# SRainGit/CAE-LO

Measured on AMD Instinct MI355X. Metric: KITTI frames/sec end-to-end (keypts+desc+match+RANSAC), higher is better.
Workload: dtype f32

## Files before the change

### cae-lo_amd/csrc/caelo_internal.h

```cpp
#pragma once
#include <hip/hip_runtime.h>
#include <stdint.h>
#include <stdio.h>
#include <string.h>

#include "../../include/caelo.h"

#define CAELO_API extern "C" __attribute__((visibility("default")))

void caelo_set_error(const char *fmt, ...);

#define CAELO_HIP(expr)                                                                     \
    do {                                                                                    \
        hipError_t _e = (expr);                                                             \
        if (_e != hipSuccess) {                                                             \
            caelo_set_error("%s:%d: %s failed: %s", __FILE__, __LINE__, #expr, hipGetErrorString(_e)); \
            return CAELO_ERR_HIP;                                                           \
        }                                                                                   \
    } while (0)

#define CAELO_LAUNCH_CHECK()                                                                \
    do {                                                                                    \
        hipError_t _e = hipGetLastError();                                                  \
        if (_e != hipSuccess) {                                                             \
            caelo_set_error("%s:%d: kernel launch failed: %s", __FILE__, __LINE__, hipGetErrorString(_e)); \
            return CAELO_ERR_HIP;                                                           \
        }                                                                                   \
    } while (0)

#define CAELO_REQUIRE(cond, msg)                         \
    do {                                                 \
        if (!(cond)) {                                   \
            caelo_set_error("%s: %s", __func__, msg);    \
            return CAELO_ERR_ARG;                        \
        }                                                \
    } while (0)

struct caelo_ctx {
    int device;
    float *resp_w;
    bool has_resp;
    float *enc_w1;
    float *enc_b1;
    float *enc_w2;
    float *enc_b2;
    float *enc_c0;
    float *enc_w3;
    float *enc_b3;
    void *enc_w1f;
    void *enc_w2x;
    void *enc_w3x;
    void *enc_wd1x;
    float *enc_bd1;
    float *enc_wd2;
    void *enc_wd2q;
    float *enc_bd2;
    void *enc32_wd1x;
    float *enc32_bd1;
    bool has_enc;
    int enc_hidden, enc_code;
    bool enc_reference;
    int32_t *faults;
    double *proj_edge;
    float *dec_w;
    bool has_dec;
    int dec_hidden, dec_out;
    double calib_angle;
};

#define CAELO_EMPTY_KEY 0xFFFFFFFFFFFFFFFFull

struct caelo_brick_table {
    unsigned long long *keys;
    unsigned long long *bits;
    uint32_t mask;
};

struct caelo_kd;
struct caelo_voxmap {
    int64_t max_points;
    caelo_kd *kd;
    bool order_tracked;
    bool kd_lists;
    caelo_brick_table brick[3];
    unsigned long long *vkeys[3];
    uint32_t *vfirst[3];
    uint32_t vmask[3];
    int32_t *counts;
    uint32_t *list0, *list1;
    unsigned long long *sp_keys, *sb_keys;
    uint32_t *sp_first, *sb_cnt;
    uint4 *sp_list;
    uint32_t sp_mask;
    size_t sp_off, sp_bytes;
    char *base;
    size_t ff_bytes_keys, ff_bytes_min, ff_bytes_all, zero_off, zero_bytes, total_bytes;
    bool lists_valid;
    void *scratch;
    int64_t scratch_bytes;
    char *xo_base;
    size_t xo_bytes;
    int xo_frames;
    float *corr;
};

void kd_destroy(caelo_voxmap *m);
void seqloader_rings(const caelo_seqloader *L, int *ring_batches, int *keep_batches);
int kd_store_lists(caelo_voxmap *m, const int16_t *const lists[3], const int64_t ns[3], hipStream_t s);
int kd_begin_device_lists(caelo_voxmap *m, int16_t *vox_out[3], int32_t **n_out, hipStream_t s);
int kd_resolve(const caelo_voxmap *m, const float *pts, int pts_ld, int64_t k_max, const int32_t *n_key, uint64_t *bits, uint8_t *flags,
               hipStream_t s);
int kd_resolve_many(int n, const caelo_voxmap *const *maps, const float *const *pts, int pts_ld, int64_t k_max, const int32_t *const *n_key,
                    uint64_t *const *bits, uint8_t *const *flags, hipStream_t s, bool queues_clear = false);
#define KD_ST_CENSUS 20
int kd_fused_storage(caelo_voxmap *m, int16_t *vox_out[3], int32_t **state_out);
int kd_report_left(int n, const caelo_voxmap *const *maps, int32_t *const *status, hipStream_t s);

struct SuspectTables {
    unsigned long long *sp_keys, *sb_keys;
    uint32_t *sp_first, *sb_cnt;
    uint4 *list;
    uint32_t mask;
};
inline SuspectTables suspect_tables(const caelo_voxmap *m) {
    return SuspectTables{m->sp_keys, m->sb_keys, m->sp_first, m->sb_cnt, m->sp_list, m->sp_mask};
}

#ifndef CAELO_FB_MAX
#define CAELO_FB_MAX 8
#endif
struct DedupScratch;
struct caelo_frame_dev {
    const float *pc;
    int64_t n;
    int32_t pc_stride, dist_c;
    float *ring;
    int32_t *counter, *winner;
    float *resp;
    unsigned long long *cand;
    int32_t *cand_count;
    unsigned long long *kp_elig;
    int64_t *key_pixels;
    float *key_pts, *valid;
    int32_t *n_key;
    uint8_t *flags;
    int32_t *status;
    int32_t kp_ld, valid_ld;
    caelo_brick_table brick[3];
    int32_t *counts;
    uint32_t *list0, *list1;
    SuspectTables sp;
    unsigned long long *vkeys[3];
    uint32_t *vfirst[3];
    uint32_t vmask0, vmask12;
    unsigned long long *bits;
    DedupScratch *dd;
};
struct caelo_frame_set {
    caelo_frame_dev f[CAELO_FB_MAX];
    int32_t n;
};
static_assert(sizeof(caelo_frame_set) <= 3800, "caelo_frame_set must fit the kernel argument segment");
void frame_dev_set_map(caelo_frame_dev &d, const caelo_voxmap *m);

struct caelo_pair_dev {
    const float *f0, *f1;
    const int32_t *n0, *n1;
    const float *pc0, *pc1;
    int64_t *pair_idx;
    void *ws_match, *ws_ransac;
    const double *rand;
    caelo_pose_result *result;
    uint8_t *mask;
    caelo_ransac_cert *cert;
    int32_t cert_only;
};
struct caelo_pair_set {
    caelo_pair_dev p[CAELO_FB_MAX];
    int32_t n;
    int32_t *faults;
};
int match_set(const caelo_pair_set &ps, int ld0, int64_t k0_max, int ld1, int64_t k1_max, int dim, hipStream_t s);
int ransac_set(const caelo_pair_set &ps, int pld0, int pld1, int64_t k1_max, hipStream_t s);
struct caelo_adaptive_table {
    const float *rows;
    const int32_t *n_key, *pairs;
    const int64_t *pair_idx;
    const double *draws;
    double threshold;
    caelo_adaptive_result *result;
    uint8_t *mask;
    int64_t n_pairs;
};
int adaptive_table(const caelo_adaptive_table &at, hipStream_t s);
int certify_record(const caelo_ransac_cert &c, const double *rnd, caelo_pose_result *res, uint8_t *mask, int64_t mask_len, int32_t *evals);

struct caelo_clear_item {
    void *ptr;
    size_t bytes;
    uint32_t pattern;
};
#define CAELO_CLEAR_MAX 12
struct caelo_clear_list {
    caelo_clear_item item[CAELO_CLEAR_MAX];
    int n;
};
int caelo_clear_many(const caelo_clear_list &list, hipStream_t s);
int caelo_clear_many_set(const caelo_clear_list *lists, int n_frames, hipStream_t s);

int ring_project_launch(caelo_ctx *c, const float *pc, int64_t n, float *ring, int32_t *counter, int32_t *winner, int32_t *status,
                        hipStream_t s);
int ring_respond_launch(caelo_ctx *c, const float *in, int in_w, int in_c, float *resp, hipStream_t s);
int ring_keypoints_launch(const float *ring, int ring_w, int ring_c, int dist_c, const int32_t *counter, int cnt_w,
                          const float *resp, unsigned long long *cand, int32_t *cand_count,
                          int64_t *key_pixels, float *key_pts, int kp_ld, float *valid, int valid_ld, int32_t *n_key,
                          int32_t *status, hipStream_t s);
int ring_project_set(caelo_ctx *c, const caelo_frame_set &fs, hipStream_t s);
int ring_respond_set(caelo_ctx *c, const caelo_frame_set &fs, int in_w, int in_c, hipStream_t s, int row0, int rows);
int ring_keypoints_set(const caelo_frame_set &fs, int ring_w, int ring_c, int cnt_w, hipStream_t s);
int ring_keypoints_select_set(const caelo_frame_set &fs, int ring_w, int ring_c, hipStream_t s);
int front_fused_set(caelo_ctx *c, caelo_voxmap *const *maps, const caelo_frame_set &fs, hipStream_t s);
void vox_clear_items(caelo_voxmap *m, int level, caelo_clear_list &list);
int vox_clear_for_fast_build(caelo_voxmap *m, caelo_clear_list &list, hipStream_t s);
int vox_clear_for_fast_build_set(caelo_voxmap *const *maps, int n, caelo_clear_list *lists, hipStream_t s);
int vox_build_fast_set(caelo_voxmap *const *maps, const caelo_frame_set &fs, hipStream_t s);
int vox_build_set(caelo_voxmap *const *maps, const caelo_frame_set &fs, bool track_order, hipStream_t s);
int vox_patches_set(const caelo_frame_set &fs, int64_t k_max, bool check_counts, hipStream_t s);
int dedup_set(const caelo_frame_set &fs, bool enabled, hipStream_t s);
int vox_build_launch(caelo_voxmap *m, const float *pc, int64_t n, int stride, bool track_order, int32_t *status,
                     hipStream_t s);
int vox_build_fast_launch(caelo_voxmap *m, const float *pc, int64_t n, int stride, int32_t *status, hipStream_t s);
int vox_patches_launch(const caelo_voxmap *m, const float *pts, int pts_ld, int64_t k_max, const int32_t *n_key,
                       uint64_t *bits, uint8_t *flags, int32_t *status, bool check_counts, hipStream_t s,
                       void *dedup_scratch = nullptr);
#define CAELO_FRAME_PATCHES (CAELO_MAX_KEYPTS * 3)
struct caelo_dedup_tables {
    int32_t count;
    int32_t pad[63];
    int32_t list[CAELO_FRAME_PATCHES];
    int32_t slot_of[CAELO_FRAME_PATCHES];
};
#define CAELO_FRAME_BITS_BYTES ((size_t)CAELO_FRAME_PATCHES * 64 * 8)
#define CAELO_FRAME_BUF_BYTES (CAELO_FRAME_BITS_BYTES + sizeof(caelo_dedup_tables))
__host__ __device__ inline caelo_dedup_tables *caelo_frame_tables(const uint64_t *frame_bits) {
    return (caelo_dedup_tables *)((char *)frame_bits + CAELO_FRAME_BITS_BYTES);
}
#define DD_SLOTS_FRAME 8192
#define DD_SLOTS_SET 65536
#define DD_EMPTY 0xFFFFFFFFFFFFFFFFull
struct DedupScratch {
    unsigned long long table[DD_SLOTS_SET];
    int32_t pslot[CAELO_FRAME_PATCHES];
    int32_t rep[CAELO_FRAME_PATCHES];
};
__host__ __device__ inline uint32_t dedup_slot_mask(int n_frames) { return (n_frames > 1 ? DD_SLOTS_SET : DD_SLOTS_FRAME) - 1; }
int64_t dedup_scratch_bytes();
void dedup_clear_item(void *scratch, int n_frames, caelo_clear_list &list);
unsigned long long dedup_hash_mask();
bool dedup_enabled(int mode);
int dedup_launch(uint64_t *frame_bits, void *scratch, bool enabled, hipStream_t s);

#define CAELO_ENC_MAX_FRAMES CAELO_FB_MAX
struct caelo_enc_out {
    float *base[CAELO_ENC_MAX_FRAMES];
    int64_t per_frame;
};
#define CAELO_ENC_WS_HEADER 4096
#define CAELO_ENC_WS_MFMA 3072
struct caelo_enc_in {
    const unsigned long long *bits;
    int64_t frame_stride;
    int32_t per_frame, n_frames, dedup;
    int32_t yield;
};
__device__ inline const caelo_dedup_tables *enc_tables(const caelo_enc_in &in, int f) {
    return (const caelo_dedup_tables *)(in.bits + (size_t)f * in.frame_stride + (size_t)in.per_frame * 64);
}
int encode_batch_impl(caelo_ctx *c, const uint64_t *bits, int64_t n_patches, int group, const caelo_enc_out &outs,
                      int out_stride, void *ws, hipStream_t s, hipEvent_t *ev, const caelo_enc_in *in = nullptr);
int64_t enc_dense_pad(int64_t n);
int enc_upload_dense1(const float *wd1, const float *bd1, int K, void **wx_dev, float **bd_dev);
int64_t enc_dense32_part_bytes(int64_t np);
void enc_dense32_slices(int64_t *used, int64_t *sized);
int enc_dense32_head_launch(caelo_ctx *c, const float *f3, int64_t n_patches, int64_t np, float *part, int group, float *out,
                            int out_stride, hipStream_t s);
int encode_impl(caelo_ctx *c, const uint64_t *bits, int64_t n_patches, int group, float *out, int out_stride, void *ws,
                hipStream_t s, hipEvent_t *ev);

struct caelo_extract_args {
    caelo_ctx *ctx;
    caelo_voxmap *map;
    const float *pc;
    int64_t n;
    int dist_channels, mode;
    float *key_pts;
    int kp_ld;
    float *features;
    int feat_ld;
    float *valid;
    int valid_ld;
    int64_t *key_pixels;
    int32_t *n_key;
    uint8_t *flags;
    int32_t *status;
    void *ws;
    uint64_t *bits;
};
int extract_check(const caelo_extract_args &a);
int extract_front_launch(const caelo_extract_args &a, hipStream_t s);
int extract_front_set(const caelo_extract_args *args, int n, hipStream_t s, hipStream_t s_vox = nullptr, hipEvent_t ev_fork = nullptr,
                      hipEvent_t ev_join = nullptr);
int extract_encode_launch(const caelo_extract_args &a, hipStream_t s);
int exact_patches_prepare(caelo_voxmap *const *maps, int n_frames);
void exact_patches_clear_item(caelo_voxmap *m, caelo_clear_list &list);
int exact_patches_redo(caelo_voxmap *const *maps, const caelo_frame_set &fs, const caelo_extract_args *args, int n, hipStream_t s);

int correct_prepare(caelo_voxmap *const *maps, int n);
int correct_set(const caelo_extract_args *args, int n, hipStream_t s);

#define CAELO_KP_HIST_BINS 2048

typedef float f32x4 __attribute__((ext_vector_type(4)));
#define MFMA16(a, b, c) __builtin_amdgcn_mfma_f32_16x16x4f32((a), (b), (c), 0, 0, 0)

__device__ inline void caelo_frame_block(int n_frames, unsigned &frame, unsigned &block, unsigned &per_frame) {
    per_frame = gridDim.x / (unsigned)n_frames;
    if ((n_frames & (n_frames - 1)) == 0) {
        frame = blockIdx.x & (unsigned)(n_frames - 1);
        block = blockIdx.x / (unsigned)n_frames;
    } else {
        frame = blockIdx.x / per_frame;
        block = blockIdx.x - frame * per_frame;
    }
}

__device__ inline void caelo_lds_barrier() { __asm__ volatile("s_waitcnt lgkmcnt(0)\n\ts_barrier" ::: "memory"); }

__host__ __device__ inline unsigned long long caelo_pack3(int x, int y, int z) {
    return ((unsigned long long)(unsigned)(x & 0xFFFFF) << 40) | ((unsigned long long)(unsigned)(y & 0xFFFFF) << 20) |
           (unsigned long long)(unsigned)(z & 0xFFFFF);
}

__device__ inline uint32_t caelo_hash64(unsigned long long k) {
    k ^= k >> 33;
    k *= 0xff51afd7ed558ccdULL;
    k ^= k >> 33;
    k *= 0xc4ceb9fe1a85ec53ULL;
    k ^= k >> 33;
    return (uint32_t)k;
}

__device__ inline unsigned long long caelo_dd_mix(unsigned long long k) {
    k ^= k >> 33;
    k *= 0xff51afd7ed558ccdULL;
    k ^= k >> 33;
    k *= 0xc4ceb9fe1a85ec53ULL;
    k ^= k >> 33;
    return k;
}
__device__ inline void caelo_dedup_insert(unsigned long long word, int lane, int p, int gp, DedupScratch *S, DedupScratch *T, uint32_t slot_mask,
                                          unsigned long long hash_mask) {
    unsigned long long h = caelo_dd_mix(word + 0x9E3779B97F4A7C15ull * (unsigned)(lane + 1));
#pragma unroll
    for (int o = 32; o > 0; o >>= 1) h += __shfl_xor(h, o);
    if (lane != 0) return;
    h = caelo_dd_mix(h) & hash_mask & 0xFFFFFFFFFEull;
    const unsigned long long mine = (h << 24) | (unsigned)gp;
    uint32_t slot = (uint32_t)caelo_dd_mix(h) & slot_mask;
    for (;;) {
        const unsigned long long cur = atomicCAS(&T->table[slot], DD_EMPTY, mine);
        if (cur == DD_EMPTY) break;
        if ((cur >> 24) == h) {
            if (mine < cur) atomicMin(&T->table[slot], mine);
            break;
        }
        slot = (slot + 1) & slot_mask;
    }
    S->pslot[p] = (int32_t)slot;
}

__device__ inline int caelo_brick_find(const caelo_brick_table &t, unsigned long long key) {
    uint32_t h = caelo_hash64(key) & t.mask;
    for (uint32_t probe = 0; probe <= t.mask; ++probe) {
        const unsigned long long k = t.keys[h];
        if (k == key) return (int)h;
        if (k == CAELO_EMPTY_KEY) return -1;
        h = (h + 1) & t.mask;
    }
    return -1;
}

static inline hipStream_t caelo_stream(void *s) { return (hipStream_t)s; }

#include <mutex>
#define CAELO_MAX_DEVICES 64
template <typename T, typename F>
static T per_device_once(int device, T (&slot)[CAELO_MAX_DEVICES], bool (&have)[CAELO_MAX_DEVICES], std::mutex &mu, F make) {
    const int d = device >= 0 && device < CAELO_MAX_DEVICES ? device : 0;
    std::lock_guard<std::mutex> lock(mu);
    if (!have[d]) { slot[d] = make(); have[d] = true; }
    return slot[d];
}

#ifdef __HIPCC__
__device__ inline int caelo_block_reserve(int32_t *gcounter, bool pred, int *s_tmp) {
    const int lane = threadIdx.x & 63;
    if (threadIdx.x == 0) s_tmp[0] = 0;
    __syncthreads();
    const unsigned long long m = __ballot(pred);
    int wbase = 0;
    if (m && lane == __ffsll((long long)m) - 1) wbase = atomicAdd(&s_tmp[0], __popcll(m));
    if (m) wbase = __shfl(wbase, __ffsll((long long)m) - 1);
    __syncthreads();
    if (threadIdx.x == 0) s_tmp[1] = s_tmp[0] ? atomicAdd(gcounter, s_tmp[0]) : 0;
    __syncthreads();
    return s_tmp[1] + wbase + __popcll(m & ((1ull << lane) - 1ull));
}
__device__ inline int caelo_block_reserve_async(int32_t *gcounter, bool pred, int *s_tmp) {
    const int lane = threadIdx.x & 63;
    if (threadIdx.x == 0) s_tmp[0] = 0;
    caelo_lds_barrier();
    const unsigned long long m = __ballot(pred);
    int wbase = 0;
    if (m && lane == __ffsll((long long)m) - 1) wbase = atomicAdd(&s_tmp[0], __popcll(m));
    if (m) wbase = __shfl(wbase, __ffsll((long long)m) - 1);
    caelo_lds_barrier();
    if (threadIdx.x == 0) s_tmp[1] = s_tmp[0] ? atomicAdd(gcounter, s_tmp[0]) : 0;
    caelo_lds_barrier();
    return s_tmp[1] + wbase + __popcll(m & ((1ull << lane) - 1ull));
}
__device__ inline void caelo_block_add(int32_t *gcounter, int value, int *s_tmp) {
    if (threadIdx.x == 0) s_tmp[0] = 0;
    __syncthreads();
#pragma unroll
    for (int o = 32; o > 0; o >>= 1) value += __shfl_xor(value, o);
    if ((threadIdx.x & 63) == 0 && value) atomicAdd(&s_tmp[0], value);
    __syncthreads();
    if (threadIdx.x == 0 && s_tmp[0]) atomicAdd(gcounter, s_tmp[0]);
}
#endif
```

### cae-lo_amd/csrc/voxel_front.inc

```
#pragma once

#define VOX_SIZE 0.02
#define BLOCK_REAL 1.28
#define VIS_L 99.84
#define VIS_W 99.84
#define VIS_H 14.72

__device__ inline int table_insert(unsigned long long *keys, uint32_t mask, unsigned long long key) {
    uint32_t h = caelo_hash64(key) & mask;
    for (uint32_t probe = 0; probe <= mask; ++probe) {
        unsigned long long k = keys[h];
        if (k == key) return (int)h;
        if (k == CAELO_EMPTY_KEY) {
            k = atomicCAS(&keys[h], CAELO_EMPTY_KEY, key);
            if (k == CAELO_EMPTY_KEY || k == key) return (int)h;
        }
        h = (h + 1) & mask;
    }
    return -1;
}

__device__ inline int table_find(const unsigned long long *keys, uint32_t mask, unsigned long long key) {
    uint32_t h = caelo_hash64(key) & mask;
    for (uint32_t probe = 0; probe <= mask; ++probe) {
        const unsigned long long k = keys[h];
        if (k == key) return (int)h;
        if (k == CAELO_EMPTY_KEY) return -1;
        h = (h + 1) & mask;
    }
    return -1;
}

__device__ inline int brick_set(caelo_brick_table t, int x, int y, int z) {
    const int slot = table_insert(t.keys, t.mask, caelo_pack3(x >> 3, y >> 3, z >> 3));
    if (slot < 0) return -1;
    const unsigned long long bit = 1ull << (((y & 7) << 3) | (z & 7));
    unsigned long long *w = &t.bits[(size_t)slot * 8 + (x & 7)];
    if (__hip_atomic_load(w, __ATOMIC_RELAXED, __HIP_MEMORY_SCOPE_AGENT) & bit) return 0;
    const unsigned long long old = atomicOr(w, bit);
    return (old & bit) ? 0 : 1;
}

__device__ inline int table_insert_new(unsigned long long *keys, uint32_t mask, unsigned long long key, bool *is_new) {
    uint32_t h = caelo_hash64(key) & mask;
    *is_new = false;
    for (uint32_t probe = 0; probe <= mask; ++probe) {
        unsigned long long k = keys[h];
        if (k == key) return (int)h;
        if (k == CAELO_EMPTY_KEY) {
            k = atomicCAS(&keys[h], CAELO_EMPTY_KEY, key);
            if (k == CAELO_EMPTY_KEY) { *is_new = true; return (int)h; }
            if (k == key) return (int)h;
        }
        h = (h + 1) & mask;
    }
    return -1;
}

__device__ inline bool brick_mark_new(caelo_brick_table t, int x, int y, int z, int *slot_out, bool *is_new) {
    const int slot = table_insert_new(t.keys, t.mask, caelo_pack3(x >> 3, y >> 3, z >> 3), is_new);
    *slot_out = slot;
    if (slot < 0) return false;
    const unsigned long long bit = 1ull << (((y & 7) << 3) | (z & 7));
    unsigned long long *w = &t.bits[(size_t)slot * 8 + (x & 7)];
    if (!(__hip_atomic_load(w, __ATOMIC_RELAXED, __HIP_MEMORY_SCOPE_AGENT) & bit))
        (void)__hip_atomic_fetch_or(w, bit, __ATOMIC_RELAXED, __HIP_MEMORY_SCOPE_AGENT);
    return true;
}

__device__ inline bool brick_mark(caelo_brick_table t, int x, int y, int z) {
    const int slot = table_insert(t.keys, t.mask, caelo_pack3(x >> 3, y >> 3, z >> 3));
    if (slot < 0) return false;
    const unsigned long long bit = 1ull << (((y & 7) << 3) | (z & 7));
    unsigned long long *w = &t.bits[(size_t)slot * 8 + (x & 7)];
    if (!(__hip_atomic_load(w, __ATOMIC_RELAXED, __HIP_MEMORY_SCOPE_AGENT) & bit))
        (void)__hip_atomic_fetch_or(w, bit, __ATOMIC_RELAXED, __HIP_MEMORY_SCOPE_AGENT);
    return true;
}

struct VoxIdx {
    int g[3];
    int v1[3];
    int v2[3];
    bool ok, oob, nonfinite;
};

__device__ inline int vox_trunc_div(double p, double d, double inv_d) {
    const double t = p * inv_d;
    const int n = (int)t;
    const double frac = fabs(t - (double)n);
    if (frac > 1e-6 && frac < 1.0 - 1e-6) return n;
    return (int)(p / d);
}

__device__ inline VoxIdx voxel_indices(float fx, float fy, float fz) {
    VoxIdx r;
    r.ok = false;
    r.oob = false;
    r.nonfinite = fx != fx || fy != fy || fz != fz;
    if (r.nonfinite) return r;
    if (fabsf(fx) > (float)VIS_L || fabsf(fy) > (float)VIS_W || fabsf(fz) > (float)VIS_H) return r;
    const double p[3] = {(double)fx + VIS_L, (double)fy + VIS_W, (double)fz + VIS_H};
#pragma unroll
    for (int a = 0; a < 3; ++a) {
        const int b = vox_trunc_div(p[a], BLOCK_REAL, 1.0 / BLOCK_REAL);
        const double rem = p[a] - b * BLOCK_REAL;
        const int v = rem >= 0.0 ? vox_trunc_div(rem, VOX_SIZE, 1.0 / VOX_SIZE) : (int)(rem / VOX_SIZE);
        if (v < 0 || v >= 64) r.oob = true;
        r.g[a] = v + b * 64;
        r.v1[a] = vox_trunc_div(p[a], VOX_SIZE * 8, 1.0 / (VOX_SIZE * 8));
        r.v2[a] = vox_trunc_div(p[a], VOX_SIZE * 32, 1.0 / (VOX_SIZE * 32));
    }
    r.ok = !r.oob;
    return r;
}

static __device__ __forceinline__ void vox_points_body(const caelo_frame_dev &F, const unsigned int block) {
    const float *__restrict__ pc = F.pc;
    const int64_t n = F.n;
    const int stride = F.pc_stride;
    const caelo_brick_table b0 = F.brick[0];
    uint32_t *list0 = F.list0;
    int32_t *counts = F.counts, *status = F.status;
    const SuspectTables sp = F.sp;
    const int64_t i = (int64_t)block * blockDim.x + threadIdx.x;
    const int lane = threadIdx.x & 63;
    VoxIdx v;
    v.ok = false;
    v.oob = false;
    v.nonfinite = false;
    if (i < n) {
        const float *p = pc + i * stride;
        v = voxel_indices(p[0], p[1], p[2]);
    }
    int st = (v.oob ? CAELO_ST_VOXEL_OOB : 0) | (v.nonfinite ? CAELO_ST_NONFINITE : 0);
    unsigned long long key = CAELO_EMPTY_KEY;
    if (i < n) F.vkeys[0][i] = v.ok ? caelo_pack3(v.g[0], v.g[1], v.g[2]) : CAELO_EMPTY_KEY;
    if (v.ok) {
        bool consistent = true;
#pragma unroll
        for (int a = 0; a < 3; ++a) consistent &= (v.v1[a] == (v.g[a] >> 3)) && (v.v2[a] == (v.g[a] >> 5));
        key = caelo_pack3(v.g[0] >> 3, v.g[1] >> 3, v.g[2] >> 3);
        if (!consistent) {
            bool sp_new = false;
            const int ss = table_insert_new(sp.sp_keys, sp.mask, caelo_pack3(v.g[0], v.g[1], v.g[2]), &sp_new);
            uint32_t sb = 0xFFFFFFFFu;
            if (sp_new) {
                sb = (uint32_t)table_insert(sp.sb_keys, sp.mask, key);
                atomicAdd(&sp.sb_cnt[sb], 1u);
            }
            sp.list[atomicAdd(&counts[6], 1)] = make_uint4((uint32_t)i, (uint32_t)ss, sb, 0u);
        }
    }
    const unsigned long long prev = __shfl_up(key, 1);
    const bool head = v.ok && (lane == 0 || prev != key);
    const uint32_t h0 = caelo_hash64(key) & b0.mask;
    unsigned long long old = CAELO_EMPTY_KEY;
    if (head) old = atomicCAS(&b0.keys[h0], CAELO_EMPTY_KEY, key);
    __shared__ int s_tmp[2];
    const int lpos = caelo_block_reserve_async(&counts[4], head, s_tmp);
    int slot = -1;
    if (head) {
        bool is_new = old == CAELO_EMPTY_KEY;
        slot = (int)h0;
        if (!is_new && old != key) slot = table_insert_new(b0.keys, b0.mask, key, &is_new);
        if (slot < 0) st |= CAELO_ST_MAP_FULL;
        list0[lpos] = is_new ? (uint32_t)slot : 0xFFFFFFFFu;
    }
    __shared__ unsigned long long s_agg[4][64][8];
    __shared__ int s_slot[4][64];
    const int wave = threadIdx.x >> 6;
    const unsigned long long heads = __ballot(head);
    const unsigned long long upto = heads & ((lane == 63) ? ~0ull : ((2ull << lane) - 1ull));
    const int run = __popcll(upto) - 1;
    const int nruns = __popcll(heads);
#pragma unroll
    for (int w = 0; w < 8; w += 2) *(ulonglong2 *)&s_agg[wave][lane][w] = make_ulonglong2(0ull, 0ull);
    if (head) s_slot[wave][run] = slot;
    __builtin_amdgcn_fence(__ATOMIC_RELEASE, "wavefront");
    __builtin_amdgcn_wave_barrier();
    __builtin_amdgcn_fence(__ATOMIC_ACQUIRE, "wavefront");
    if (v.ok) atomicOr(&s_agg[wave][run][v.g[0] & 7], 1ull << (((v.g[1] & 7) << 3) | (v.g[2] & 7)));
    __builtin_amdgcn_fence(__ATOMIC_RELEASE, "wavefront");
    __builtin_amdgcn_wave_barrier();
    __builtin_amdgcn_fence(__ATOMIC_ACQUIRE, "wavefront");
    {
        const int w = lane & 7;
        for (int r = lane >> 3; r < nruns; r += 8) {
            const unsigned long long bitsw = s_agg[wave][r][w];
            const int sl = s_slot[wave][r];
            if (bitsw && sl >= 0)
                (void)__hip_atomic_fetch_or(&b0.bits[(size_t)sl * 8 + w], bitsw, __ATOMIC_RELAXED, __HIP_MEMORY_SCOPE_AGENT);
        }
    }
    if (st) atomicOr(status, st);
}

#define SUSPECT_LDS 128
static __device__ __forceinline__ void vox_suspects_first(const caelo_frame_dev &F, int block) {
    const int nsp = F.counts[6];
    if (nsp == 0) return;
    __shared__ unsigned long long s_key[SUSPECT_LDS];
    __shared__ uint32_t s_slot[SUSPECT_LDS];
    const bool listed = nsp <= SUSPECT_LDS;
    if (listed) {
        if ((int)threadIdx.x < nsp) {
            const uint32_t ss = F.sp.list[threadIdx.x].y;
            s_slot[threadIdx.x] = ss;
            s_key[threadIdx.x] = F.sp.sp_keys[ss];
        }
        __syncthreads();
    }
    const int64_t i = (int64_t)block * blockDim.x + threadIdx.x;
    if (i >= F.n) return;
    const unsigned long long key = F.vkeys[0][i];
    if (key == CAELO_EMPTY_KEY) return;
    if (listed) {
        for (int e = 0; e < nsp; ++e)
            if (s_key[e] == key) { atomicMin(&F.sp.sp_first[s_slot[e]], (uint32_t)i); break; }
    } else {
        const int ss = table_find(F.sp.sp_keys, F.sp.mask, key);
        if (ss >= 0) atomicMin(&F.sp.sp_first[ss], (uint32_t)i);
    }
}

#define COARSE_WGS 256
static __device__ __forceinline__ void vox_coarse_body(const caelo_frame_dev &F, const unsigned int block) {
    if (block >= COARSE_WGS) {
        vox_suspects_first(F, (int)block - COARSE_WGS);
        return;
    }
    const caelo_brick_table b0 = F.brick[0], b1 = F.brick[1];
    const uint32_t *list0 = F.list0;
    uint32_t *list1 = F.list1;
    int32_t *counts = F.counts, *status = F.status;
    const SuspectTables sp = F.sp;
    __shared__ int s_tmp[2];
    const int nb = counts[4];
    const bool any_suspect = counts[6] > 0;
    int pop = 0;
    for (int i0 = block * blockDim.x; i0 < nb; i0 += COARSE_WGS * blockDim.x) {
        const int i = i0 + threadIdx.x;
        bool is_new = false;
        int slot1 = -1;
        const uint32_t slot = i < nb ? list0[i] : 0xFFFFFFFFu;
        if (slot != 0xFFFFFFFFu) {
            const unsigned long long k = b0.keys[slot];
            const ulonglong2 *w = (const ulonglong2 *)(b0.bits + (size_t)slot * 8);
            int mine = 0;
#pragma unroll
            for (int q = 0; q < 4; ++q) { const ulonglong2 u = w[q]; mine += __popcll(u.x) + __popcll(u.y); }
            pop += mine;
            if (any_suspect) {
                const int sb = table_find(sp.sb_keys, sp.mask, k);
                if (sb >= 0) mine -= (int)(sp.sb_cnt[sb] + 1u);
            }
            const int x = (int)((k >> 40) & 0xFFFFF), y = (int)((k >> 20) & 0xFFFFF), z = (int)(k & 0xFFFFF);
            if (mine > 0 && !brick_mark_new(b1, x, y, z, &slot1, &is_new)) atomicOr(status, CAELO_ST_MAP_FULL);
        }
        const int lpos = caelo_block_reserve(&counts[5], is_new, s_tmp);
        if (is_new) list1[lpos] = (uint32_t)slot1;
    }
    caelo_block_add(&counts[0], pop, s_tmp);
}

static __device__ __forceinline__ void vox_coarse2_body(const caelo_frame_dev &F, const unsigned int block, const unsigned int nblocks) {
    const caelo_brick_table b1 = F.brick[1], b2 = F.brick[2];
    const uint32_t *list1 = F.list1;
    int32_t *counts = F.counts, *status = F.status;
    __shared__ int s_tmp[2];
    const int nb = counts[5];
    int pop = 0, pop2 = 0;
    for (int i = block * blockDim.x + threadIdx.x; i < nb; i += nblocks * blockDim.x) {
        const uint32_t slot = list1[i];
        const unsigned long long k = b1.keys[slot];
        const int bx = (int)((k >> 40) & 0xFFFFF) << 3, by = (int)((k >> 20) & 0xFFFFF) << 3, bz = (int)(k & 0xFFFFF) << 3;
        const unsigned long long *w = b1.bits + (size_t)slot * 8;
        unsigned long long orv[2] = {0ull, 0ull};
#pragma unroll
        for (int hx = 0; hx < 2; ++hx) {
            const unsigned long long m = w[4 * hx] | w[4 * hx + 1] | w[4 * hx + 2] | w[4 * hx + 3];
            pop += __popcll(w[4 * hx]) + __popcll(w[4 * hx + 1]) + __popcll(w[4 * hx + 2]) + __popcll(w[4 * hx + 3]);
#pragma unroll
            for (int hy = 0; hy < 2; ++hy)
#pragma unroll
                for (int hz = 0; hz < 2; ++hz) {
                    const unsigned long long sel = (0x0F0F0F0Full << (4 * hz)) << (32 * hy);
                    const int y2 = (by >> 2) + hy, z2 = (bz >> 2) + hz;
                    if (m & sel) orv[hx] |= 1ull << (((y2 & 7) << 3) | (z2 & 7));
                }
        }
        if (orv[0] | orv[1]) {
            const int x2 = bx >> 2;
            const int slot2 = table_insert(b2.keys, b2.mask, caelo_pack3(x2 >> 3, by >> 5, bz >> 5));
            if (slot2 < 0) atomicOr(status, CAELO_ST_MAP_FULL);
            else {
#pragma unroll
                for (int hx = 0; hx < 2; ++hx) {
                    if (!orv[hx]) continue;
                    unsigned long long *wd = &b2.bits[(size_t)slot2 * 8 + ((x2 + hx) & 7)];
                    if ((__hip_atomic_load(wd, __ATOMIC_RELAXED, __HIP_MEMORY_SCOPE_AGENT) & orv[hx]) != orv[hx]) {
                        const unsigned long long old = __hip_atomic_fetch_or(wd, orv[hx], __ATOMIC_RELAXED, __HIP_MEMORY_SCOPE_AGENT);
                        pop2 += __popcll(orv[hx] & ~old);
                    }
                }
            }
        }
    }
    caelo_block_add(&counts[1], pop, s_tmp);
    __syncthreads();
    caelo_block_add(&counts[2], pop2, s_tmp);
}

#define COARSE2_WGS 64

static __device__ __forceinline__ void vox_suspects_resolve_body(const caelo_frame_dev &F, const unsigned int block, const unsigned int nblocks) {
    const float *__restrict__ pc = F.pc;
    const int stride = F.pc_stride;
    const caelo_brick_table b1 = F.brick[1], b2 = F.brick[2];
    uint32_t *list1 = F.list1;
    int32_t *counts = F.counts, *status = F.status;
    const SuspectTables sp = F.sp;
    const int nsp = counts[6];
    for (int e = block * blockDim.x + threadIdx.x; e < nsp; e += nblocks * blockDim.x) {
        const uint4 ent = sp.list[e];
        const uint32_t j = sp.sp_first[ent.y];
        const float *p = pc + (int64_t)j * stride;
        const VoxIdx v = voxel_indices(p[0], p[1], p[2]);
        bool is_new = false;
        const int s1 = table_insert_new(b1.keys, b1.mask, caelo_pack3(v.v1[0] >> 3, v.v1[1] >> 3, v.v1[2] >> 3), &is_new);
        if (s1 < 0) atomicOr(status, CAELO_ST_MAP_FULL);
        else {
            if (is_new) list1[atomicAdd(&counts[5], 1)] = (uint32_t)s1;
            const unsigned long long bit = 1ull << (((v.v1[1] & 7) << 3) | (v.v1[2] & 7));
            if (!(atomicOr(&b1.bits[(size_t)s1 * 8 + (v.v1[0] & 7)], bit) & bit)) atomicAdd(&counts[1], 1);
        }
        const int r2 = brick_set(b2, v.v2[0], v.v2[1], v.v2[2]);
        if (r2 < 0) atomicOr(status, CAELO_ST_MAP_FULL);
        else if (r2) atomicAdd(&counts[2], 1);
    }
}
```

Before: 19760.

## Aggregate coarse brick marks per wavefront and stage suspect keys in LDS

The coarse voxel pass now groups lanes whose bricks map to the same parent brick. One leader per group does the hash-table insert, and the group's occupancy bits are merged in a per-wave LDS image before a single global atomic OR per word. Suspect brick keys and counts are staged into LDS when few enough, replacing a hash probe per brick with a linear scan. The list and suspect loads are issued early, barriers use a lighter LDS-only form, and the status OR is deferred to one atomic per thread. These changes target contention on global atomics and hash probing, at the cost of extra wave-level sync and more complex control flow.

```diff
diff --git a/cae-lo_amd/csrc/caelo_internal.h b/cae-lo_amd/csrc/caelo_internal.h
--- a/cae-lo_amd/csrc/caelo_internal.h
+++ b/cae-lo_amd/csrc/caelo_internal.h
@@ -438,4 +438,13 @@
     __syncthreads();
     if (threadIdx.x == 0 && s_tmp[0]) atomicAdd(gcounter, s_tmp[0]);
 }
+__device__ inline void caelo_block_add_async(int32_t *gcounter, int value, int *s_tmp) {
+    if (threadIdx.x == 0) s_tmp[0] = 0;
+    caelo_lds_barrier();
+#pragma unroll
+    for (int o = 32; o > 0; o >>= 1) value += __shfl_xor(value, o);
+    if ((threadIdx.x & 63) == 0 && value) atomicAdd(&s_tmp[0], value);
+    caelo_lds_barrier();
+    if (threadIdx.x == 0 && s_tmp[0]) atomicAdd(gcounter, s_tmp[0]);
+}
 #endif
diff --git a/cae-lo_amd/csrc/voxel_front.inc b/cae-lo_amd/csrc/voxel_front.inc
--- a/cae-lo_amd/csrc/voxel_front.inc
+++ b/cae-lo_amd/csrc/voxel_front.inc
@@ -225,6 +225,7 @@
 }
 
 #define COARSE_WGS 256
+#define COARSE_RUNS 16
 static __device__ __forceinline__ void vox_coarse_body(const caelo_frame_dev &F, const unsigned int block) {
     if (block >= COARSE_WGS) {
         vox_suspects_first(F, (int)block - COARSE_WGS);
@@ -236,32 +237,124 @@
     int32_t *counts = F.counts, *status = F.status;
     const SuspectTables sp = F.sp;
     __shared__ int s_tmp[2];
+    __shared__ unsigned long long s_sbkey[SUSPECT_LDS];
+    __shared__ uint32_t s_sbcnt[SUSPECT_LDS];
+    __shared__ unsigned long long s_agg[4][COARSE_RUNS][8];
+    __shared__ int s_slot[4][COARSE_RUNS];
+    int i0 = block * blockDim.x;
+    uint32_t slot = (uint32_t)i0 + threadIdx.x <= b0.mask ? list0[i0 + threadIdx.x] : 0xFFFFFFFFu;
+    uint32_t sbz = threadIdx.x < SUSPECT_LDS && threadIdx.x < (sp.mask + 1u) / 3u ? sp.list[threadIdx.x].z : 0xFFFFFFFFu;
     const int nb = counts[4];
-    const bool any_suspect = counts[6] > 0;
-    int pop = 0;
-    for (int i0 = block * blockDim.x; i0 < nb; i0 += COARSE_WGS * blockDim.x) {
-        const int i = i0 + threadIdx.x;
+    const int nsp = counts[6];
+    __asm__ volatile("" ::"s"(nb), "s"(nsp));
+    if (i0 >= nb) return;
+    const bool listed = nsp > 0 && nsp <= SUSPECT_LDS;
+    const int lane = threadIdx.x & 63, wave = threadIdx.x >> 6;
+    if (i0 + (int)threadIdx.x >= nb) slot = 0xFFFFFFFFu;
+    if (!listed || (int)threadIdx.x >= nsp) sbz = 0xFFFFFFFFu;
+    bool staged = !listed;
+    int pop = 0, st = 0;
+    for (;;) {
+        const bool brick = slot != 0xFFFFFFFFu;
+        const uint32_t slot_or_0 = brick ? slot : 0u;
+        const unsigned long long k = b0.keys[slot_or_0];
+        ulonglong2 u[4];
+        {
+            const ulonglong2 *w = (const ulonglong2 *)(b0.bits + (size_t)slot_or_0 * 8);
+#pragma unroll
+            for (int q = 0; q < 4; ++q) u[q] = w[q];
+        }
+        unsigned long long sk = CAELO_EMPTY_KEY;
+        uint32_t sc = 0u;
+        if (!staged) {
+            const uint32_t sbi = sbz != 0xFFFFFFFFu ? sbz : 0u;
+            sk = sp.sb_keys[sbi];
+            sc = sp.sb_cnt[sbi];
+        }
+        if (!staged) {
+            if ((int)threadIdx.x < nsp) {
+                s_sbkey[threadIdx.x] = sbz != 0xFFFFFFFFu ? sk : CAELO_EMPTY_KEY;
+                s_sbcnt[threadIdx.x] = sc + 1u;
+            }
+            caelo_lds_barrier();
+            staged = true;
+        }
+        int mine = 0;
+        if (brick) {
+#pragma unroll
+            for (int q = 0; q < 4; ++q) mine += __popcll(u[q].x) + __popcll(u[q].y);
+            pop += mine;
+            if (nsp > 0) {
+                if (listed) {
+                    int held = 0;
+#pragma unroll 4
+                    for (int e = 0; e < nsp; ++e) held = s_sbkey[e] == k ? (int)s_sbcnt[e] : held;
+                    mine -= held;
+                } else {
+                    const int sb = table_find(sp.sb_keys, sp.mask, k);
+                    if (sb >= 0) mine -= (int)(sp.sb_cnt[sb] + 1u);
+                }
+            }
+        }
+        const bool live = brick && mine > 0;
+        const int x = (int)((k >> 40) & 0xFFFFF), y = (int)((k >> 20) & 0xFFFFF), z = (int)(k & 0xFFFFF);
+        const unsigned long long key1 = caelo_pack3(x >> 3, y >> 3, z >> 3);
+        unsigned long long rem = __ballot(live);
+        int run = -1, leader = 0, nruns = 0;
+        while (rem) {
+            const int l = __ffsll(rem) - 1;
+            const unsigned long long lk = ((unsigned long long)(uint32_t)__builtin_amdgcn_readlane((int)(key1 >> 32), l) << 32) |
+                                          (uint32_t)__builtin_amdgcn_readlane((int)(uint32_t)key1, l);
+            const bool same = live && key1 == lk;
+            if (same) { run = nruns; leader = l; }
+            rem &= ~__ballot(same);
+            ++nruns;
+        }
+        const bool head = live && lane == leader;
+        const uint32_t h1 = caelo_hash64(key1) & b1.mask;
+        unsigned long long old = CAELO_EMPTY_KEY;
+        if (head) old = atomicCAS(&b1.keys[h1], CAELO_EMPTY_KEY, key1);
+        static_assert(COARSE_RUNS * 8 == 64 * 2, "each lane clears two words of its wavefront's image");
+        *(ulonglong2 *)&s_agg[wave][lane >> 2][(lane & 3) * 2] = make_ulonglong2(0ull, 0ull);
         bool is_new = false;
         int slot1 = -1;
-        const uint32_t slot = i < nb ? list0[i] : 0xFFFFFFFFu;
-        if (slot != 0xFFFFFFFFu) {
-            const unsigned long long k = b0.keys[slot];
-            const ulonglong2 *w = (const ulonglong2 *)(b0.bits + (size_t)slot * 8);
-            int mine = 0;
-#pragma unroll
-            for (int q = 0; q < 4; ++q) { const ulonglong2 u = w[q]; mine += __popcll(u.x) + __popcll(u.y); }
-            pop += mine;
-            if (any_suspect) {
-                const int sb = table_find(sp.sb_keys, sp.mask, k);
-                if (sb >= 0) mine -= (int)(sp.sb_cnt[sb] + 1u);
+        if (head) {
+            is_new = old == CAELO_EMPTY_KEY;
+            slot1 = (int)h1;
+            if (!is_new && old != key1) slot1 = table_insert_new(b1.keys, b1.mask, key1, &is_new);
+            if (slot1 < 0) st |= CAELO_ST_MAP_FULL;
+        }
+        const int rslot = __shfl(slot1, leader);
+        if (head && run < COARSE_RUNS) s_slot[wave][run] = slot1;
+        __builtin_amdgcn_fence(__ATOMIC_RELEASE, "wavefront");
+        __builtin_amdgcn_wave_barrier();
+        __builtin_amdgcn_fence(__ATOMIC_ACQUIRE, "wavefront");
+        if (live) {
+            const unsigned long long bit = 1ull << (((y & 7) << 3) | (z & 7));
+            if (run < COARSE_RUNS) atomicOr(&s_agg[wave][run][x & 7], bit);
+            else if (rslot >= 0)
+                (void)__hip_atomic_fetch_or(&b1.bits[(size_t)rslot * 8 + (x & 7)], bit, __ATOMIC_RELAXED, __HIP_MEMORY_SCOPE_AGENT);
+        }
+        __builtin_amdgcn_fence(__ATOMIC_RELEASE, "wavefront");
+        __builtin_amdgcn_wave_barrier();
+        __builtin_amdgcn_fence(__ATOMIC_ACQUIRE, "wavefront");
+        {
+            const int w = lane & 7, nimg = nruns < COARSE_RUNS ? nruns : COARSE_RUNS;
+            for (int r = lane >> 3; r < nimg; r += 8) {
+                const unsigned long long bitsw = s_agg[wave][r][w];
+                const int sl = s_slot[wave][r];
+                if (bitsw && sl >= 0)
+                    (void)__hip_atomic_fetch_or(&b1.bits[(size_t)sl * 8 + w], bitsw, __ATOMIC_RELAXED, __HIP_MEMORY_SCOPE_AGENT);
             }
-            const int x = (int)((k >> 40) & 0xFFFFF), y = (int)((k >> 20) & 0xFFFFF), z = (int)(k & 0xFFFFF);
-            if (mine > 0 && !brick_mark_new(b1, x, y, z, &slot1, &is_new)) atomicOr(status, CAELO_ST_MAP_FULL);
-        }
-        const int lpos = caelo_block_reserve(&counts[5], is_new, s_tmp);
+        }
+        const int lpos = caelo_block_reserve_async(&counts[5], is_new, s_tmp);
         if (is_new) list1[lpos] = (uint32_t)slot1;
-    }
-    caelo_block_add(&counts[0], pop, s_tmp);
+        i0 += COARSE_WGS * blockDim.x;
+        if (i0 >= nb) break;
+        slot = i0 + (int)threadIdx.x < nb ? list0[i0 + threadIdx.x] : 0xFFFFFFFFu;
+    }
+    caelo_block_add_async(&counts[0], pop, s_tmp);
+    if (st) atomicOr(status, st);
 }
 
 static __device__ __forceinline__ void vox_coarse2_body(const caelo_frame_dev &F, const unsigned int block, const unsigned int nblocks) {
```

Result: no change. 19640 (median of 2 runs) (-0.6%).
